# DoHoonKim8/stark-verifier

Hardware: AMD Instinct MI355X
Metric: recursive plonky2 proofs/sec (Semaphore d=20) (higher is better)
Workload: dtype u64 (Goldilocks field, integer); 1 GPU; recursive: per unit one Semaphore signal (group 2^20, n=2^13, blowup 8, 28 FRI queries, 16 PoW bits, zk) + the recursive proof verifying it (n=2^14, same FRI parameters); 128 units per GPU per step, 10 prover contexts per GPU; all_gather of (nullifier|topic) + Poseidon aggregation root per step; parallelism=independent proofs sharded over ranks, no data-path collective, exchange=none (one rank): gl355_aggregation_root over the local leaves, units_proven_in_process=1674

## Files before the change

stark-verifier_amd/csrc/gl355_internal.h:

```cpp
#pragma once
#include <hip/hip_runtime.h>
#include <stdint.h>
#include <string.h>

#include <algorithm>
#include <map>
#include <mutex>
#include <string>
#include <vector>

#include "../../include/gl355.h"
#include "gl_field.cuh"
#include "merkle_common.cuh"
#include "coset_interp.h"

namespace gl355 { struct Ctx; }

struct gl355_oracle {
    struct gl355::Ctx* ctx;
    uint32_t log_n, rate_bits, batch, leaf_len, cap_height;
    uint64_t* coeffs;
    uint64_t* lde;
    uint64_t* digests;
    uint64_t* cap;
    uint64_t n_digests;
    int32_t hasher;
};

namespace gl355 {

struct Ctx;

#define GL355_HIP(ctx, expr)                                                          \
    do {                                                                              \
        hipError_t _e = (expr);                                                       \
        if (_e != hipSuccess) return (ctx)->fail_hip(_e, #expr, __FILE__, __LINE__);  \
    } while (0)
#define GL355_TRY(expr)          \
    do {                         \
        int32_t _rc = (expr);    \
        if (_rc != GL355_OK) return _rc; \
    } while (0)
#define LAUNCH_CHECK(ctx) GL355_HIP(ctx, hipGetLastError())

struct Ctx {
    int device = 0;
    hipStream_t stream = nullptr;
    bool own_stream = false;
    bool external_stream = false;
    std::string err;
    uint64_t* tw_fwd = nullptr;
    uint64_t* tw_inv = nullptr;
    const uint64_t* twr(uint32_t rho, bool inv) const { return tw_fwd + 32768 + ((rho - 3) * 2 + (inv ? 1 : 0)) * 32768; }
    hipEvent_t ev0 = nullptr, ev1 = nullptr;

    struct PowTab { uint64_t* lo; uint64_t* hi; };
    std::map<std::vector<uint64_t>, PowTab> pow_cache;
    std::map<std::vector<uint64_t>, uint64_t*> full_cache;
    int32_t full_pow_table(const uint64_t* lo, const uint64_t* hi, uint32_t n_cosets, uint32_t log_n, const uint64_t** out);
    int32_t full_step_table(const uint64_t* lo, const uint64_t* hi, uint32_t l1, uint32_t l2, bool inv, const uint64_t** out);
    int32_t nat_step_table(const uint64_t* lo, const uint64_t* hi, uint32_t l1, uint32_t l2, const uint64_t** out);
    int32_t l24_mid_table(const uint64_t** out);

    struct Block { void* p; size_t size; bool used; uint64_t serial; };
    std::vector<Block> blocks;
    uint64_t block_serial = 0;

    struct ProfRec { const char* name; hipEvent_t e0, e1; uint64_t bytes; };
    uint32_t replay_threads = 1;
    uint32_t batch_units = 8;
    uint32_t ntt_single_pass_max_log = 12;
    int blocking_sync = 0;
    hipEvent_t sync_ev = nullptr;
    hipError_t wait();
    hipError_t wait_impl();
    hipError_t d2h(void* dst, const void* src, size_t bytes);
    uint64_t wait_ns = 0, wait_calls = 0;
    uint64_t wait_cpu_ns = 0, prove_cpu_ns = 0, prove_calls = 0;
    uint32_t merkle_lanes_log = 14;
    uint32_t leaf_lanes_log = 16;
    bool prof_on = false;
    std::vector<ProfRec> prof;
    std::vector<hipEvent_t> ev_pool;
    hipEvent_t prof_event();

    int32_t fail(int32_t code, const char* msg);
    int32_t fail_hip(hipError_t e, const char* expr, const char* file, int line);
    int32_t alloc(size_t bytes, void** out);
    void release(void* p);
    void* pinned_buf = nullptr;
    size_t pinned_size = 0;
    int32_t pinned(size_t bytes, void** out);
    void* rt_rows[2] = {nullptr, nullptr};
    void* rt_drows[2] = {nullptr, nullptr};
    void* rt_aux[2] = {nullptr, nullptr};
    size_t rt_bytes = 0, rt_aux_bytes = 0;
    bool device_replay = true;
    hipStream_t rt_copy_stream = nullptr;
    int32_t runtime_buffers(size_t bytes, size_t aux_bytes, uint64_t* rows[2], uint64_t* drows[2], void* aux[2], hipStream_t* copy_stream);
    void runtime_buffers_free();
    void release_all();
    void trim_since(uint64_t mark);
    int32_t pow_tables_multi(const std::vector<uint64_t>& bases, const uint64_t** lo, const uint64_t** hi);
    int32_t pow_tables(uint64_t base, const uint64_t** lo, const uint64_t** hi) {
        return pow_tables_multi(std::vector<uint64_t>{gl_canon(base)}, lo, hi);
    }
};

struct ProfScope {
    Ctx* ctx; int idx = -1;
    ProfScope(Ctx* c, const char* name, uint64_t alg_bytes = 0) : ctx(c) {
        if (!c->prof_on) return;
        Ctx::ProfRec r{name, c->prof_event(), c->prof_event(), alg_bytes};
        if (!r.e0 || !r.e1) return;
        (void)hipEventRecord(r.e0, c->stream);
// ... 264 lines not shown
```

stark-verifier_amd/csrc/merkle.hip:

```cpp
#include "gl355_internal.h"
#include "poseidon.cuh"
#include "merkle_common.cuh"

namespace gl355 {


struct PoseidonHasher {
    static constexpr bool wide_digests = true;
    static GL_DEV void permute(uint64_t (&s)[12]) { psd_permute(s); }
    static GL_DEV uint64_t out(uint64_t x) { return gl_canon(x); }
    static GL_DEV uint64_t in2(uint64_t x) { return x; }
};

__global__ void __launch_bounds__(256) poseidon_permute_kernel(uint64_t* states, uint64_t count) { permute_body<PoseidonHasher>(states, count); }

constexpr int psd_leaf_waves = 4;
__global__ void __launch_bounds__(256) __attribute__((amdgpu_waves_per_eu(psd_leaf_waves))) hash_leaves_kernel(LeafArgs a) { hash_leaves_body<PoseidonHasher>(a); }

__global__ void __launch_bounds__(256) merkle_level_kernel(uint64_t* digests, uint64_t* cap, uint32_t sub_bits,
                                                          uint32_t layer, uint64_t n_nodes ) {
    merkle_level_body<PoseidonHasher>(digests, cap, sub_bits, layer, n_nodes);
}

__device__ __constant__ const uint32_t PSD_CIRC_DEV[12] = {17, 15, 41, 16, 2, 28, 13, 13, 39, 18, 34, 20};
// ... 219 lines not shown
#undef GL355_WIDE_LEAVES
        GL355_HIP(ctx, hipGetLastError());
    }
    return merkle_build_above_leaves(ctx, n_groups, sub_bits, digests, cap);
}

int32_t merkle_build_above_leaves(Ctx* ctx, uint64_t n_leaves, uint32_t sub_bits, uint64_t* digests, uint64_t* cap) {
    const uint64_t lanes_max = 1ull << ctx->merkle_lanes_log;
    const uint32_t top_levels_max = (n_leaves >> sub_bits) < 64 ? 6 : MERKLE_TOP_LEVELS;
    const bool fast_lanes = (n_leaves >> sub_bits) < 64;
    uint32_t top_levels = std::min<uint32_t>(top_levels_max, sub_bits);
    while (top_levels > 1 && ((n_leaves >> (sub_bits - top_levels + 1)) > lanes_max)) top_levels--;
    uint32_t top_from = sub_bits + 1;
    if (top_levels >= 1 && ((n_leaves >> (sub_bits - top_levels + 1)) <= lanes_max)) top_from = sub_bits - top_levels + 1;
    for (uint32_t layer = 1; layer <= sub_bits; layer++) {
        const uint64_t n_nodes = n_leaves >> layer;
        if (layer == top_from) {
            ProfScope ps(ctx, "merkle_top_kernel", (2 * n_nodes - (n_leaves >> sub_bits)) * 96);
            if (fast_lanes) hipLaunchKernelGGL(merkle_top_kernel<3>, dim3((uint32_t)(n_leaves >> sub_bits)), dim3(1024), 0, ctx->stream, digests, cap, sub_bits, layer, top_levels);
            else hipLaunchKernelGGL(merkle_top_kernel<0>, dim3((uint32_t)(n_leaves >> sub_bits)), dim3(1024), 0, ctx->stream, digests, cap, sub_bits, layer, top_levels);
            GL355_HIP(ctx, hipGetLastError());
            break;
        }
        ProfScope ps(ctx, n_nodes <= lanes_max ? "merkle_level_lanes_kernel" : "merkle_level_kernel", n_nodes * 96);
        if (n_nodes <= lanes_max) {
            if (fast_lanes) hipLaunchKernelGGL(merkle_level_lanes_kernel<3>, dim3((uint32_t)((n_nodes + 3) / 4)), dim3(64), 0, ctx->stream,
                                               digests, cap, sub_bits, layer, n_nodes);
            else hipLaunchKernelGGL(merkle_level_lanes_kernel<0>, dim3((uint32_t)((n_nodes + 3) / 4)), dim3(64), 0, ctx->stream,
                                    digests, cap, sub_bits, layer, n_nodes);
        } else {
            hipLaunchKernelGGL(merkle_level_kernel, dim3((uint32_t)((n_nodes + 255) / 256)), dim3(256), 0, ctx->stream,
                               digests, cap, sub_bits, layer, n_nodes);
        }
        GL355_HIP(ctx, hipGetLastError());
    }
    return GL355_OK;
}

int32_t pow_grind_units_dev(Ctx* ctx, int32_t hasher, uint32_t B, const uint64_t* states, const uint32_t* pos, uint32_t bits, uint64_t start, uint64_t* landing,
                            uint64_t* const* witness_host) {
    if (bits > 40) return ctx->fail(GL355_E_UNSUPPORTED, "pow: more than 40 bits of grinding refused");
    const HasherLaunch& h = launch_of(hasher);
    PowArgs pa;
    memset(&pa, 0, sizeof pa);
    for (uint32_t u = 0; u < B; u++) {
        for (int k = 0; k < 12; k++) pa.state[u * 12 + k] = gl_canon(states[u * 12 + k]);
        pa.pos[u] = pos[u]; pa.todo[u] = 1;
    }
    Scratch pb(ctx);
    GL355_TRY(pb.get(GL355_MAX_UNITS * 8));
    pa.best = reinterpret_cast<unsigned long long*>(pb.p);
    pa.bits = bits;
    GL355_HIP(ctx, hipMemsetAsync(pb.p, 0xFF, GL355_MAX_UNITS * 8, ctx->stream));
    uint64_t per_launch = 1ull << std::min<uint32_t>(std::max<uint32_t>(bits + 1, 12), h.grind_window_log);
    uint64_t base = start;
    for (uint32_t left = B; left;) {
        ProfScope ps(ctx, h.grind_scope, 0);
        pa.start = base;
        hipLaunchKernelGGL(h.grind, dim3((uint32_t)(per_launch / 256), B), dim3(256), 0, ctx->stream, pa);
        GL355_HIP(ctx, hipGetLastError());
        GL355_HIP(ctx, ctx->d2h(landing, pb.p, (uint64_t)B * 8));
        GL355_HIP(ctx, ctx->wait());
        for (uint32_t u = 0; u < B; u++)
            if (pa.todo[u] && landing[u] != ~0ull) { *witness_host[u] = landing[u]; pa.todo[u] = 0; left--; }
        base += per_launch;
        if (per_launch < (1ull << h.grind_window_log)) per_launch <<= 1;
        if (base - start > (1ull << 44)) return ctx->fail(GL355_E_UNSUPPORTED, "pow: no witness found in 2^44 candidates");
    }
    return GL355_OK;
}

int32_t pow_grind_dev(Ctx* ctx, int32_t hasher, const uint64_t state[12], uint32_t pos, uint32_t bits, uint64_t start,
                      uint64_t* witness_host) {
    if (pos >= 8) return ctx->fail(GL355_E_INVALID_ARG, "pow: witness position must be in the rate part");
    uint64_t landing;
    return pow_grind_units_dev(ctx, hasher, 1, state, &pos, bits, start, &landing, &witness_host);
}

}
```

stark-verifier_amd/csrc/merkle_common.cuh:

```cuda
#pragma once
#include <stdint.h>
#include <hip/hip_runtime.h>

#include "../../include/gl355.h"
#include "gl_field.cuh"

namespace gl355 {

__host__ __device__ __forceinline__ uint64_t digest_slot(uint32_t layer, uint64_t k) {
    return 2 * (((k >> 1) << (layer + 1)) + (1ull << layer) - 1) + (k & 1);
}

__device__ __forceinline__ uint64_t* leaf_digest_dst(uint64_t* out, uint64_t* cap, uint32_t linear, uint32_t sub_bits, uint64_t i) {
    if (linear) return out + i * 4;
    if (sub_bits == 0) return cap + i * 4;
    const uint64_t sub_leaves = 1ull << sub_bits;
    const uint64_t t = i >> sub_bits, k = i & (sub_leaves - 1);
    return out + (t * 2 * (sub_leaves - 1) + digest_slot(0, k)) * 4;
}

struct MerkleNode {
    uint64_t* tree; uint64_t* cap; uint32_t sub_bits, layer; uint64_t t, k;
    __device__ __forceinline__ uint64_t child() const { return digest_slot(layer - 1, 2 * k); }
    __device__ __forceinline__ uint64_t* dst() const { return (layer == sub_bits) ? cap + t * 4 : tree + digest_slot(layer, k) * 4; }
};
__device__ __forceinline__ MerkleNode merkle_node(uint64_t* digests, uint64_t* cap, uint32_t sub_bits, uint32_t layer, uint64_t t, uint64_t k) {
    const uint64_t sub_leaves = 1ull << sub_bits;
    return {digests + t * 2 * (sub_leaves - 1) * 4, cap, sub_bits, layer, t, k};
}
__device__ __forceinline__ MerkleNode merkle_node(uint64_t* digests, uint64_t* cap, uint32_t sub_bits, uint32_t layer, uint64_t g) {
    const uint64_t per = (1ull << sub_bits) >> layer;
    return merkle_node(digests, cap, sub_bits, layer, g / per, g % per);
}

struct LeafArgs {
    const uint64_t* leaves;
    uint64_t n_leaves;
    uint32_t leaf_len;
    uint32_t col_major;
    uint64_t stride;
    uint64_t* out;
    uint32_t sub_bits;
    uint32_t linear;
    uint32_t always_hash;
    uint64_t* cap;
    uint32_t unit_log;
    uint32_t n_main;
    uint64_t unit_stride;
    const uint64_t* salt;
    uint64_t salt_unit_stride;
};

__device__ __forceinline__ uint64_t leaf_elem(const LeafArgs& a, uint64_t g, uint32_t k) {
    if (a.unit_log == 0) return a.col_major ? a.leaves[(uint64_t)k * a.stride + g] : a.leaves[g * a.stride + k];
    const uint64_t u = g >> a.unit_log, i = g & ((1ull << a.unit_log) - 1);
    if (k < a.n_main) {
        const uint64_t* base = a.leaves + u * a.unit_stride;
        return a.col_major ? base[(uint64_t)k * a.stride + i] : base[i * a.stride + k];
    }
    return a.salt[u * a.salt_unit_stride + (uint64_t)(k - a.n_main) * a.stride + i];
}

struct PowArgs { uint64_t state[GL355_MAX_UNITS * 12]; uint32_t pos[GL355_MAX_UNITS]; uint32_t todo[GL355_MAX_UNITS]; uint32_t bits; uint64_t start; unsigned long long* best; };

#if defined(__HIPCC__)
#define GL_WAVE_LDS_SYNC()                                      \
    do {                                                        \
        __builtin_amdgcn_fence(__ATOMIC_SEQ_CST, "wavefront");  \
        __builtin_amdgcn_wave_barrier();                        \
    } while (0)

template <class H> GL_DEV void store_digest(uint64_t* dst, const uint64_t (&d)[4]) {
    if constexpr (H::wide_digests) {
        *reinterpret_cast<ulonglong2*>(dst) = make_ulonglong2(d[0], d[1]);
        *reinterpret_cast<ulonglong2*>(dst + 2) = make_ulonglong2(d[2], d[3]);
    } else {
#pragma unroll
        for (int k = 0; k < 4; k++) dst[k] = d[k];
    }
}

template <class H> GL_DEV void permute_body(uint64_t* states, uint64_t count) {
    const uint64_t i = blockIdx.x * (uint64_t)blockDim.x + threadIdx.x;
    if (i >= count) return;
    uint64_t s[12];
#pragma unroll
    for (int k = 0; k < 12; k++) s[k] = states[i * 12 + k];
    H::permute(s);
#pragma unroll
    for (int k = 0; k < 12; k++) states[i * 12 + k] = H::out(s[k]);
}

template <class H> GL_DEV void hash_leaves_body(const LeafArgs& a) {
    const uint64_t i = blockIdx.x * (uint64_t)blockDim.x + threadIdx.x;
    if (i >= a.n_leaves) return;
    uint64_t s[12];
#pragma unroll
    for (int k = 0; k < 12; k++) s[k] = 0;
    const uint32_t len = a.leaf_len;
    uint64_t d[4];
    if (len <= 4 && !a.always_hash) {
        for (uint32_t k = 0; k < 4; k++) {
            uint64_t v = 0;
            if (k < len) v = leaf_elem(a, i, k);
            d[k] = gl_canon(v);
        }
    } else {
#pragma unroll 1
        for (uint32_t off = 0; off < len; off += 8) {
            const uint32_t m = min(8u, len - off);
#pragma unroll
            for (uint32_t k = 0; k < 8; k++) {
                if (k < m) s[k] = leaf_elem(a, i, off + k);
            }
            H::permute(s);
        }
#pragma unroll
        for (int k = 0; k < 4; k++) d[k] = H::out(s[k]);
    }
    store_digest<H>(leaf_digest_dst(a.out, a.cap, a.linear, a.sub_bits, i), d);
}

template <class H> GL_DEV void merkle_level_body(uint64_t* digests, uint64_t* cap, uint32_t sub_bits, uint32_t layer, uint64_t n_nodes ) {
    const uint64_t g = blockIdx.x * (uint64_t)blockDim.x + threadIdx.x;
    if (g >= n_nodes) return;
    const MerkleNode nd = merkle_node(digests, cap, sub_bits, layer, g);
    const uint64_t* in = nd.tree + nd.child() * 4;
    uint64_t s[12];
    if constexpr (H::wide_digests) {
        const ulonglong2 l0 = *reinterpret_cast<const ulonglong2*>(in);
        const ulonglong2 l1 = *reinterpret_cast<const ulonglong2*>(in + 2);
        const ulonglong2 r0 = *reinterpret_cast<const ulonglong2*>(in + 4);
        const ulonglong2 r1 = *reinterpret_cast<const ulonglong2*>(in + 6);
        s[0] = l0.x; s[1] = l0.y; s[2] = l1.x; s[3] = l1.y; s[4] = r0.x; s[5] = r0.y; s[6] = r1.x; s[7] = r1.y;
    } else {
#pragma unroll
        for (int e = 0; e < 8; e++) s[e] = in[e];
    }
#pragma unroll
    for (int e = 8; e < 12; e++) s[e] = 0;
    H::permute(s);
    const uint64_t d[4] = {H::out(s[0]), H::out(s[1]), H::out(s[2]), H::out(s[3])};
    store_digest<H>(nd.dst(), d);
}

template <class H> GL_DEV void two_to_one_body(const uint64_t* l, const uint64_t* r, uint64_t n, uint64_t* out) {
    const uint64_t i = blockIdx.x * (uint64_t)blockDim.x + threadIdx.x;
    if (i >= n) return;
    uint64_t s[12] = {H::in2(l[4 * i]), H::in2(l[4 * i + 1]), H::in2(l[4 * i + 2]), H::in2(l[4 * i + 3]),
                      H::in2(r[4 * i]), H::in2(r[4 * i + 1]), H::in2(r[4 * i + 2]), H::in2(r[4 * i + 3]), 0, 0, 0, 0};
    H::permute(s);
#pragma unroll
    for (int k = 0; k < 4; k++) out[4 * i + k] = H::out(s[k]);
}

template <class H> GL_DEV void pow_grind_units_body(const PowArgs& a) {
    const uint32_t u = blockIdx.y;
    if (!a.todo[u]) return;
    const uint64_t w = a.start + blockIdx.x * (uint64_t)blockDim.x + threadIdx.x;
    if (w > __hip_atomic_load(a.best + u, __ATOMIC_RELAXED, __HIP_MEMORY_SCOPE_AGENT)) return;
    uint64_t s[12];
#pragma unroll
    for (int k = 0; k < 12; k++) s[k] = a.state[u * 12 + k];
#pragma unroll
    for (int k = 0; k < 12; k++) if ((uint32_t)k == a.pos[u]) s[k] = w;
    H::permute(s);
    const uint64_t resp = H::out(s[7]);
    if (a.bits == 0 || (resp >> (64 - a.bits)) == 0) atomicMin(a.best + u, (unsigned long long)w);
}
#endif

}
```

stark-verifier_amd/csrc/prover_batch.hip:

```cpp
#include "gl355_internal.h"
#include "blinding.cuh"
#include "poseidon.cuh"

using namespace gl355;

namespace gl355 {

struct BOracle {
    Ctx* ctx = nullptr;
    uint32_t B = 0, log_n = 0, rate_bits = 0, batch = 0, leaf_len = 0, cap_height = 0;
    uint64_t* base = nullptr;
    uint64_t *coeffs = nullptr, *lde = nullptr, *salt = nullptr, *digests = nullptr, *cap = nullptr;
    uint64_t n_dig = 0;
    ~BOracle() { if (base && ctx) ctx->release(base); }
    int32_t alloc(Ctx* c, uint32_t b, uint32_t lg, uint32_t rb, uint32_t bat, bool salted, uint32_t cap_h) {
        ctx = c; B = b; log_n = lg; rate_bits = rb; batch = bat; leaf_len = bat + (salted ? GL355_SALT_SIZE : 0); cap_height = cap_h;
        const uint64_t n = 1ull << lg, N = n << rb, n_cap = 1ull << cap_h;
        n_dig = 2 * (N - n_cap);
        const uint64_t total = (uint64_t)B * ((uint64_t)bat * n + (uint64_t)leaf_len * N + n_dig * 4 + n_cap * 4);
        void* p = nullptr;
        GL355_TRY(c->alloc(total * 8, &p));
        base = reinterpret_cast<uint64_t*>(p);
        coeffs = base;
        lde = coeffs + (uint64_t)B * bat * n;
// ... 14 lines not shown

struct UnitKeys { BlindKey k[MAXB]; };

__global__ void witness_rows_units_kernel(uint64_t* wires, uint64_t n, uint32_t num_wires, const uint32_t* row_idx, const uint64_t* row_vals,
                                          uint32_t n_rows) {
    const uint64_t g = blockIdx.x * (uint64_t)blockDim.x + threadIdx.x;
    const uint64_t per = (uint64_t)n_rows * num_wires;
    if (g >= per) return;
    const uint32_t u = blockIdx.y, r = g / num_wires, c = g % num_wires;
    wires[((uint64_t)u * num_wires + c) * n + row_idx[r]] = gl_canon(row_vals[(uint64_t)u * per + g]);
}
__global__ void witness_blind_units_kernel(uint64_t* wires, uint64_t n, uint32_t num_wires, uint32_t num_routed, uint32_t blind_start, uint32_t n_blind,
                                           uint32_t z_start, uint32_t n_z_pairs, UnitKeys keys) {
    const uint64_t b = blockIdx.x * (uint64_t)blockDim.x + threadIdx.x;
    const uint64_t n_a = (uint64_t)n_blind * num_wires, n_z = (uint64_t)n_z_pairs * num_routed;
    if (4 * b >= n_a + n_z) return;
    const uint32_t u = blockIdx.y;
    uint64_t* w = wires + (uint64_t)u * num_wires * n;
    uint64_t e[4];
    blind_block_elements(keys.k[u], GL355_BLIND_STREAM_WITNESS, (uint32_t)b, e);
#pragma unroll
    for (int j = 0; j < 4; j++) {
        const uint64_t g = 4 * b + j;
        if (g < n_a) {
            const uint32_t c = g / n_blind, r = g % n_blind;
            w[(uint64_t)c * n + blind_start + r] = e[j];
        } else if (g < n_a + n_z) {
            const uint64_t h = g - n_a, c = h / n_z_pairs, k = h % n_z_pairs;
            w[c * n + z_start + 2 * k] = e[j];
            w[c * n + z_start + 2 * k + 1] = e[j];
        }
    }
}
__global__ void salt_units_kernel(uint64_t* salt, uint32_t lde_bits, UnitKeys keys, uint32_t stream) {
    const uint64_t b = blockIdx.x * (uint64_t)blockDim.x + threadIdx.x;
    const uint64_t N = 1ull << lde_bits, cnt = (uint64_t)GL355_SALT_SIZE * N;
    if (4 * b >= cnt) return;
    const uint32_t u = blockIdx.y;
    uint64_t e[4];
    blind_block_elements(keys.k[u], stream, (uint32_t)b, e);
#pragma unroll
    for (int j = 0; j < 4; j++) {
        const uint64_t g = 4 * b + j;
        const uint64_t c = g >> lde_bits, i = g & (N - 1);
        const uint64_t r = __brevll(i) >> (64 - lde_bits);
        salt[((uint64_t)u * GL355_SALT_SIZE + c) * N + r] = e[j];
    }
}

struct ZsArgs {
    const uint64_t* wires; uint64_t wires_us;
    const uint64_t* sigmas; const uint64_t* k_is;
    uint32_t log_n, n_routed, max_degree, nch, n_chunks, npp;
    uint64_t g;
    uint64_t* chunk_q;
    uint64_t* row_prod;
    uint64_t* zbuf; uint64_t z_us;
    UnitVals betas, gammas;
};
constexpr int ZS_MAX_CHUNKS = 16;
__global__ void __launch_bounds__(256) zs_rows_units_kernel(ZsArgs a) {
    const uint64_t n = 1ull << a.log_n;
    const uint64_t i = blockIdx.x * (uint64_t)blockDim.x + threadIdx.x;
    if (i >= n) return;
    const uint32_t inst = blockIdx.y, u = inst / a.nch, k = inst % a.nch;
    const uint64_t beta = a.betas.v[u * 4 + k], gamma = a.gammas.v[u * 4 + k];
    const uint64_t* wires = a.wires + (uint64_t)u * a.wires_us;
    const uint64_t x = gl_pow(a.g, i);
    const uint64_t bx = gl_mul(beta, x);
    uint64_t num[ZS_MAX_CHUNKS], pre[ZS_MAX_CHUNKS], den[ZS_MAX_CHUNKS];
    uint64_t run = 1;
#pragma unroll
    for (int ch = 0; ch < ZS_MAX_CHUNKS; ch++) {
        num[ch] = 1; den[ch] = 1; pre[ch] = run;
        if ((uint32_t)ch < a.n_chunks) {
            uint64_t nm = 1, dn = 1;
            for (uint32_t j = ch * a.max_degree; j < (ch + 1) * a.max_degree && j < a.n_routed; j++) {
                const uint64_t w = wires[(uint64_t)j * n + i];
                nm = gl_mul(nm, gl_add(gl_add(w, gl_mul(bx, a.k_is[j])), gamma));
                dn = gl_mul(dn, gl_add(gl_add(w, gl_mul(beta, a.sigmas[(uint64_t)j * n + i])), gamma));
            }
            num[ch] = nm; den[ch] = dn;
            run = gl_mul(run, dn);
        }
    }
    uint64_t inv = gl_inv(run);
    uint64_t rp = 1;
    uint64_t* cq = a.chunk_q + (uint64_t)inst * a.n_chunks * n;
#pragma unroll
    for (int ch = ZS_MAX_CHUNKS - 1; ch >= 0; ch--) {
        if ((uint32_t)ch < a.n_chunks) {
            const uint64_t dinv = gl_mul(inv, pre[ch]);
            inv = gl_mul(inv, den[ch]);
            const uint64_t q = gl_mul(num[ch], dinv);
            cq[(uint64_t)ch * n + i] = q;
            rp = gl_mul(rp, q);
        }
    }
    a.row_prod[(uint64_t)inst * n + i] = rp;
}
__global__ void __launch_bounds__(1024) zs_scan_units_kernel(ZsArgs a) {
    __shared__ uint64_t sh[1024];
    const int tid = threadIdx.x;
    const uint32_t inst = blockIdx.x, u = inst / a.nch, k = inst % a.nch;
    const uint64_t n = 1ull << a.log_n;
    const uint64_t* row_prod = a.row_prod + (uint64_t)inst * n;
    uint64_t* z = a.zbuf + (uint64_t)u * a.z_us + (uint64_t)k * n;
    uint64_t running = 1;
    for (uint64_t base = 0; base < n; base += 1024) {
        const uint64_t i = base + tid;
        uint64_t v = i < n ? row_prod[i] : 1;
        sh[tid] = v;
        __syncthreads();
        for (int s = 1; s < 1024; s <<= 1) {
            uint64_t o = tid >= s ? sh[tid - s] : 1;
            __syncthreads();
            v = gl_mul(v, o);
            sh[tid] = v;
            __syncthreads();
        }
        const uint64_t excl = tid ? sh[tid - 1] : 1;
// ... 7 lines not shown
    const uint64_t n = 1ull << a.log_n;
    const uint64_t i = blockIdx.x * (uint64_t)blockDim.x + threadIdx.x;
    if (i >= n) return;
    const uint32_t inst = blockIdx.y, u = inst / a.nch, k = inst % a.nch;
    uint64_t* zu = a.zbuf + (uint64_t)u * a.z_us;
    const uint64_t* cq = a.chunk_q + (uint64_t)inst * a.n_chunks * n;
    uint64_t* pp = zu + ((uint64_t)a.nch + (uint64_t)k * a.npp) * n;
    uint64_t acc = zu[(uint64_t)k * n + i];
    for (uint32_t ch = 0; ch + 1 < a.n_chunks; ch++) {
        acc = gl_mul(acc, cq[(uint64_t)ch * n + i]);
        pp[(uint64_t)ch * n + i] = gl_canon(acc);
    }
}

static int32_t commit_units(Ctx* ctx, int32_t hasher, BOracle& o, bool is_coeffs, bool canonical, const UnitKeys* keys, uint32_t stream_id) {
    const uint64_t n = 1ull << o.log_n, N = n << o.rate_bits;
    const uint32_t cols = o.B * o.batch, lde_bits = o.log_n + o.rate_bits;
    if (!is_coeffs) GL355_TRY(ntt_dev(ctx, o.coeffs, o.log_n, cols, n, true, 0));
    else if (!canonical) GL355_TRY(canon_dev(ctx, o.coeffs, (uint64_t)cols * n));
    GL355_TRY(lde_dev(ctx, o.coeffs, n, o.log_n, o.rate_bits, GL355_COSET_SHIFT, cols, o.lde, N, true));
    if (o.salt) {
        const uint64_t cnt = (uint64_t)GL355_SALT_SIZE * N;
        ProfScope ps(ctx, "salt", cnt * 8 * o.B);
        hipLaunchKernelGGL(salt_units_kernel, dim3((uint32_t)((cnt / 4 + 255) / 256), o.B), dim3(256), 0, ctx->stream, o.salt, lde_bits, *keys, stream_id);
        LAUNCH_CHECK(ctx);
    }
    LeafArgs a;
    memset(&a, 0, sizeof a);
    a.leaves = o.lde; a.n_leaves = (uint64_t)o.B * N; a.leaf_len = o.leaf_len; a.col_major = 1; a.stride = N;
    a.unit_log = lde_bits; a.n_main = o.batch; a.unit_stride = (uint64_t)o.batch * N; a.salt = o.salt; a.salt_unit_stride = (uint64_t)GL355_SALT_SIZE * N;
    return merkle_build_args(ctx, hasher, a, lde_bits - o.cap_height, o.digests, o.cap);
}

int32_t observe_caps_units(Ctx* ctx, uint32_t B, uint64_t n_cap, const uint64_t* d_caps, uint64_t* stage, gl355_challenger* ch, uint64_t* const* dst) {
    GL355_HIP(ctx, ctx->d2h(stage, d_caps, (uint64_t)B * n_cap * 32));
    GL355_HIP(ctx, ctx->wait());
    for (uint32_t u = 0; u < B; u++) {
        memcpy(dst[u], stage + (uint64_t)u * n_cap * 4, n_cap * 32);
        gl355_challenger_observe(&ch[u], dst[u], n_cap * 4);
    }
    return GL355_OK;
}

static int32_t zs_units_dev(Ctx* ctx, uint32_t B, uint32_t nch, const uint64_t* wires, uint64_t wires_us, const uint64_t* sigmas, const uint64_t* k_is,
                            uint32_t log_n, uint32_t routed, uint32_t max_degree, const UnitVals& betas, const UnitVals& gammas, uint64_t* zbuf, uint64_t z_us) {
    const uint64_t n = 1ull << log_n;
    const uint32_t n_inst = B * nch, n_chunks = (routed + max_degree - 1) / max_degree;
    Scratch zs_tmp(ctx);
    GL355_TRY(zs_tmp.get((uint64_t)n_inst * (n_chunks + 1) * n * 8));
    ZsArgs za;
    memset(&za, 0, sizeof za);
    za.wires = wires; za.wires_us = wires_us; za.sigmas = sigmas; za.k_is = k_is;
    za.log_n = log_n; za.n_routed = routed; za.max_degree = max_degree; za.nch = nch; za.n_chunks = n_chunks; za.npp = n_chunks - 1;
    za.g = gl_root_of_unity(log_n);
    za.chunk_q = zs_tmp.as<uint64_t>(); za.row_prod = za.chunk_q + (uint64_t)n_inst * n_chunks * n;
    za.zbuf = zbuf; za.z_us = z_us;
    for (uint32_t i = 0; i < MAXB * 4; i++) { za.betas.v[i] = gl_canon(betas.v[i]); za.gammas.v[i] = gl_canon(gammas.v[i]); }
    ProfScope ps(ctx, "zs_partial_products", (uint64_t)n_inst * ((uint64_t)routed * n * 16 + (uint64_t)n_chunks * n * 8));
    const uint32_t blocks = (uint32_t)((n + 255) / 256);
    hipLaunchKernelGGL(zs_rows_units_kernel, dim3(blocks, n_inst), dim3(256), 0, ctx->stream, za);
    LAUNCH_CHECK(ctx);
    hipLaunchKernelGGL(zs_scan_units_kernel, dim3(n_inst), dim3(1024), 0, ctx->stream, za);
    LAUNCH_CHECK(ctx);
    hipLaunchKernelGGL(zs_partials_units_kernel, dim3(blocks, n_inst), dim3(256), 0, ctx->stream, za);
    LAUNCH_CHECK(ctx);
    return GL355_OK;
}
int32_t zs_partial_products_dev(Ctx* ctx, const uint64_t* wires, const uint64_t* sigmas, const uint64_t* k_is, uint32_t log_n, uint32_t n_routed,
                                uint32_t max_degree, uint64_t beta, uint64_t gamma, uint64_t* z_out, uint64_t* pp_out) {
    const uint64_t n = 1ull << log_n;
    const uint32_t n_chunks = (n_routed + max_degree - 1) / max_degree;
    if (n_chunks > ZS_MAX_CHUNKS) return ctx->fail(GL355_E_UNSUPPORTED, "zs_partial_products: at most 16 partial-product chunks");
    Scratch zb(ctx);
    GL355_TRY(zb.get((uint64_t)n_chunks * n * 8));
    UnitVals betas, gammas;
    memset(&betas, 0, sizeof betas); memset(&gammas, 0, sizeof gammas);
    betas.v[0] = beta; gammas.v[0] = gamma;
    GL355_TRY(zs_units_dev(ctx, 1, 1, wires, 0, sigmas, k_is, log_n, n_routed, max_degree, betas, gammas, zb.as<uint64_t>(), (uint64_t)n_chunks * n));
    GL355_HIP(ctx, hipMemcpyAsync(z_out, zb.p, n * 8, hipMemcpyDeviceToDevice, ctx->stream));
    if (n_chunks > 1) GL355_HIP(ctx, hipMemcpyAsync(pp_out, zb.as<uint64_t>() + n, (uint64_t)(n_chunks - 1) * n * 8, hipMemcpyDeviceToDevice, ctx->stream));
    return GL355_OK;
}

struct ProveRun {
    Ctx* ctx; const gl355_prover_data* pd; const gl355_circuit& c; const gl355_oracle* cs; const ProveUnit* io;
    const uint32_t B, nch, qdf, npp, routed, nw, z_width, lde_bits, cap_h, L, nq_idx;
    const uint64_t n, N, n_cap;
    const int32_t hasher; const bool zk;
    const ProofLayout lay;
    std::vector<gl355_challenger> ch;
    std::vector<uint64_t*> out;
    std::vector<uint64_t> q_idx;
    UnitKeys keys;
    UnitVals pi_hashes;
    uint64_t* stage = nullptr;
    BOracle o_w, o_z, o_q;
    OView views[4];
    PolySet all, zsset;
    UnitVals betas, gammas, alphas, zetas, fri_alpha;
    Scratch wires_keep;
    Staged s_sig, s_k;
    Scratch evb, colsA, colsB, fri_vals, ob;
    uint64_t *d_idx = nullptr, *d_open = nullptr;
    uint64_t off_leaf[4], off_sib[4], off_ev = 0, off_fsib = 0, open_words = 0;

    ProveRun(Ctx* cx, const gl355_prover_data* p, uint32_t b, const ProveUnit* units)
        : ctx(cx), pd(p), c(*p->circuit), cs(p->constants_sigmas), io(units), B(b), nch(c.num_challenges), qdf(c.max_degree), npp(c.num_partial_products),
// ... 274 lines not shown
```

stark-verifier_amd/csrc/quotient.hip:

```cpp
#include "gl355_internal.h"
#include "poseidon.cuh"

namespace gl355 {

struct QuotArgs {
    gl355_circuit c;
    const uint64_t* cs;
    const uint64_t* wires;
    const uint64_t* zs;
    uint64_t lde_stride;
    uint32_t qbits;
    const uint64_t* k_is;
    const uint64_t* xw_lo;
    const uint64_t* xw_hi;
    uint64_t zh_inv[16];
    uint64_t zh[16];
    uint64_t n_inv;
    uint64_t* out;
    const uint64_t* alpha_pw;
    uint32_t pw_stride;
    uint64_t wires_us, zs_us;
    uint64_t betas[GL355_MAX_UNITS * 4], gammas[GL355_MAX_UNITS * 4], pi_hash[GL355_MAX_UNITS * 4];
};

typedef const __attribute__((address_space(4))) uint64_t* PwTable;
template <int NCH>
struct AlphaAcc {
    uint64_t acc[NCH];
    PwTable tab;
    uint32_t stride, idx;
    GL_DEV void init(const QuotArgs& a, uint32_t unit, uint32_t first = 0) {
#pragma unroll
        for (int c = 0; c < NCH; c++) acc[c] = 0;
        tab = (PwTable)(a.alpha_pw + (uint64_t)unit * NCH * a.pw_stride); stride = a.pw_stride; idx = first;
    }
    GL_DEV void push(uint64_t term) {
#pragma unroll
        for (int c = 0; c < NCH; c++) acc[c] = gl_add(acc[c], gl_mul(term, tab[c * stride + idx]));
        idx++;
    }
    GL_DEV void push_at(uint64_t term, uint32_t k) {
#pragma unroll
        for (int c = 0; c < NCH; c++) acc[c] = gl_add(acc[c], gl_mul(term, tab[c * stride + k]));
    }
};
template <int NCH>
struct LazyAcc : AlphaAcc<NCH> {
    GL_DEV uint64_t value(int c) const { return this->acc[c]; }
};
template <>
struct LazyAcc<2> {
    uint64_t A0[2], A1[2], A2[2];
    uint32_t k0[2], k1[2], k2[2];
    PwTable tab;
    uint32_t stride, idx;
    GL_DEV void init(const QuotArgs& a, uint32_t unit, uint32_t first = 0) {
#pragma unroll
        for (int c = 0; c < 2; c++) { A0[c] = A1[c] = A2[c] = 0; k0[c] = k1[c] = k2[c] = 0; }
        tab = (PwTable)(a.alpha_pw + (uint64_t)unit * 2 * a.pw_stride); stride = a.pw_stride; idx = first;
    }
    GL_DEV void push(uint64_t term) {
        const uint64_t ax = tab[idx], ay = tab[stride + idx];
        const uint32_t t0 = (uint32_t)term, t1 = (uint32_t)(term >> 32);
        uint64_t c0, c1, c2, c3;
        asm("v_mad_u64_u32 %0, %12, %16, %18, %0\n\t"
            "v_mad_u64_u32 %1, %13, %16, %20, %1\n\t"
            "v_mad_u64_u32 %2, %14, %16, %19, %2\n\t"
            "v_mad_u64_u32 %3, %15, %16, %21, %3\n\t"
            "v_addc_co_u32_e64 %6, vcc, 0, %6, %12\n\t"
            "v_addc_co_u32_e64 %7, vcc, 0, %7, %13\n\t"
// ... 339 lines not shown
    uint32_t brk = s.degree, ni = 0;
    for (uint32_t i0 = 0; i0 < s.n; i0 += 4) {
        uint64_t v[8];
#pragma unroll
        for (int k = 0; k < 8; k++) v[k] = nx[k];
        wire_group<8>(w, 1 + 2 * (i0 + 4), last, nx);
#pragma unroll
        for (int k = 0; k < 4; k++) {
            const uint32_t i = i0 + k;
            if (i == brk) {
                uint64_t ie[2], ip[2];
                wire_group<2>(w, s.start_int + 2 * ni, s.start_int + 2 * ni + 1, ie);
                wire_group<2>(w, s.start_int + 2 * (s.n_int + ni), s.start_int + 2 * (s.n_int + ni) + 1, ip);
                push2(g, gl2_sub(gl2_make(ie[0], ie[1]), eval));
                push2(g, gl2_sub(gl2_make(ip[0], ip[1]), prod));
                eval = gl2_make(ie[0], ie[1]); prod = gl2_make(ip[0], ip[1]);
                ni++; brk += s.degree - 1;
            }
            const gl2 xm = gl2_make(gl_sub(x.c0, xs[i * stride]), x.c1);
            const gl2 vw = gl2_mul_base(gl2_make(v[2 * k], v[2 * k + 1]), ws[i]);
            eval = gl2_add(gl2_mul(eval, xm), gl2_mul(vw, prod));
            prod = gl2_mul(prod, xm);
        }
    }
    push2(g, gl2_sub(gl2_make(pv[2], pv[3]), eval));
}

template <int NCH, bool STAGE = false, bool INTERP = false>
__global__ void __launch_bounds__(STAGE ? 64 : 128) __attribute__((amdgpu_waves_per_eu(STAGE ? 1 : 3, 3))) quotient_kernel(QuotArgs a) {
    extern __shared__ __attribute__((aligned(16))) uint64_t wire_lds[];
    const uint64_t nq = 1ull << a.qbits;
    const uint64_t t = blockIdx.x * (uint64_t)blockDim.x + threadIdx.x;
    if (t >= nq) return;
    const uint32_t unit = blockIdx.y;
    const uint64_t* __restrict__ wglob = a.wires + (uint64_t)unit * a.wires_us;
    WireSrc w{wglob, a.lde_stride, t, a.lde_stride};
    if constexpr (STAGE) {
        for (uint32_t j = 0; j < a.c.num_wires; j++) wire_lds[j * 64 + threadIdx.x] = wglob[(uint64_t)j * a.lde_stride + t];
        w = WireSrc{wire_lds, 64, threadIdx.x, a.lde_stride};
    }
    const uint64_t* __restrict__ zs = a.zs + (uint64_t)unit * a.zs_us;
    const uint32_t qdb = a.qbits - a.c.degree_bits;
    const uint64_t iq = __brevll(t) >> (64 - a.qbits);
    const uint64_t x = gl_mul_small(gl_mul(a.xw_lo[iq & 4095], a.xw_hi[iq >> 12]), 7);
    const uint64_t iq_next = (iq + (1ull << qdb)) & (nq - 1);
    const uint64_t t_next = __brevll(iq_next) >> (64 - a.qbits);
    constexpr uint32_t nch = NCH;
    const uint32_t npp = a.c.num_partial_products;
    const uint32_t routed = a.c.num_routed_wires, chunk = a.c.max_degree;
    const uint32_t n_sel = a.c.num_selectors, n_cst = a.c.num_constants;

    AlphaAcc<NCH> total;
    total.init(a, unit);
    const uint64_t zh = a.zh[iq & ((1u << qdb) - 1)];
    const uint64_t l0 = gl_mul(gl_mul(zh, a.n_inv), gl_inv(gl_sub(x, 1)));
    for (uint32_t c = 0; c < nch; c++) {
        const uint64_t z = zs[(uint64_t)c * a.lde_stride + t];
        total.push(gl_sub(gl_mul(l0, z), l0));
    }
    {
        const uint32_t n_chunks = (routed + chunk - 1) / chunk;
        uint64_t prev[NCH], bx[NCH];
#pragma unroll
        for (int c = 0; c < NCH; c++) {
            prev[c] = zs[(uint64_t)c * a.lde_stride + t];
            bx[c] = gl_mul(a.betas[unit * 4 + c], x);
        }
        const uint32_t first = total.idx;
        const uint32_t sig0 = n_sel + n_cst;
        uint64_t wn = WIRE(0), sn = CONST(sig0), kn = a.k_is[0];
        for (uint32_t ch = 0; ch < n_chunks; ch++) {
            uint64_t num[NCH], den[NCH];
#pragma unroll
            for (int c = 0; c < NCH; c++) { num[c] = 1; den[c] = 1; }
            for (uint32_t j = ch * chunk; j < (ch + 1) * chunk && j < routed; j++) {
                const uint64_t wj = wn, sj = sn, kj = kn;
                const uint32_t jn = j + 1 < routed ? j + 1 : routed - 1;
                wn = WIRE(jn); sn = CONST(sig0 + jn); kn = a.k_is[jn];
                if constexpr (NCH == 2) {
                    const uint64_t a1[4] = {bx[0], bx[1], a.betas[unit * 4], a.betas[unit * 4 + 1]}, b1[4] = {kj, kj, sj, sj};
                    uint64_t p1[4], p2[4];
                    gl_mul_multi<4>(a1, b1, p1);
                    const uint64_t wg0 = gl_add(wj, a.gammas[unit * 4]), wg1 = gl_add(wj, a.gammas[unit * 4 + 1]);
                    const uint64_t a2[4] = {num[0], num[1], den[0], den[1]};
                    const uint64_t b2[4] = {gl_add(wg0, p1[0]), gl_add(wg1, p1[1]), gl_add(wg0, p1[2]), gl_add(wg1, p1[3])};
                    gl_mul_multi<4>(a2, b2, p2);
                    num[0] = p2[0]; num[1] = p2[1]; den[0] = p2[2]; den[1] = p2[3];
                } else {
#pragma unroll
                    for (int c = 0; c < NCH; c++) {
                        const uint64_t wg = gl_add(wj, a.gammas[unit * 4 + c]);
                        num[c] = gl_mul(num[c], gl_add(wg, gl_mul(bx[c], kj)));
                        den[c] = gl_mul(den[c], gl_add(wg, gl_mul(a.betas[unit * 4 + c], sj)));
                    }
                }
            }
#pragma unroll
            for (int c = 0; c < NCH; c++) {
                const uint64_t next = (ch + 1 < n_chunks) ? zs[(uint64_t)(nch + c * npp + ch) * a.lde_stride + t]
                                                          : zs[(uint64_t)c * a.lde_stride + t_next];
                total.push_at(gl_sub(gl_mul(prev[c], num[c]), gl_mul(next, den[c])), first + c * n_chunks + ch);
                prev[c] = next;
            }
        }
        total.idx = first + nch * n_chunks;
    }
    uint64_t gate_sum[NCH];
#pragma unroll
    for (int c = 0; c < NCH; c++) gate_sum[c] = 0;
    for (uint32_t gi = 0; gi < a.c.num_gates; gi++) {
        const gl355_gate gt = a.c.gates[gi];
        if (gt.type == GL355_GATE_NOOP) continue;
        GateAccT<NCH> g;
        WireSrc wg = w;
        uint64_t tg = t;
        asm volatile("" : "+s"(wg.stride), "+s"(wg.cs_stride), "+v"(tg));
        wg.idx = STAGE ? w.idx : tg;
        g.init(a, unit, total.idx);
        bool interp = false;
        if constexpr (INTERP) {
            if (gt.type == GL355_GATE_COSET_INTERPOLATION) { gate_coset_interpolation(a, wg, tg, g, gt.param); interp = true; }
        }
        if (!interp) switch (gt.type) {
            case GL355_GATE_POSEIDON: gate_poseidon(a, wg, tg, g); break;
            case GL355_GATE_BASE_SUM: gate_base_sum(a, wg, tg, g, gt.param); break;
            case GL355_GATE_CONSTANT: gate_constant(a, wg, tg, g, gt.param); break;
            case GL355_GATE_PUBLIC_INPUT: gate_public_input(a, wg, tg, g, unit); break;
            case GL355_GATE_ARITHMETIC: gate_arithmetic(a, wg, tg, g, gt.param); break;
            case GL355_GATE_ARITHMETIC_EXT: gate_arithmetic_ext(a, wg, tg, g, gt.param); break;
            case GL355_GATE_MUL_EXT: gate_mul_ext(a, wg, tg, g, gt.param); break;
            case GL355_GATE_POSEIDON_MDS: gate_poseidon_mds(a, wg, tg, g); break;
            case GL355_GATE_RANDOM_ACCESS: gate_random_access(a, wg, tg, g, gt.param); break;
            case GL355_GATE_REDUCING: gate_reducing<false>(a, wg, tg, g, gt.param); break;
            case GL355_GATE_REDUCING_EXT: gate_reducing<true>(a, wg, tg, g, gt.param); break;
            default: break;
        }
        const uint64_t sel = CONST(gt.selector_index);
        uint64_t filter = 1;
        for (uint32_t k = gt.group_start; k < gt.group_end; k++)
            if (k != gi) filter = gl_mul(filter, gl_sub(k, sel));
        if (n_sel > 1) filter = gl_mul(filter, gl_sub(0xFFFFFFFFull, sel));
#pragma unroll
        for (uint32_t c = 0; c < nch; c++) gate_sum[c] = gl_add(gate_sum[c], gl_mul(filter, g.value(c)));
    }
    const uint64_t zh_inv = a.zh_inv[iq & ((1u << qdb) - 1)];
    for (uint32_t c = 0; c < nch; c++) {
        const uint64_t v = gl_mul(gl_add(total.acc[c], gate_sum[c]), zh_inv);
        a.out[((uint64_t)unit * nch + c) * nq + t] = gl_canon(v);
    }
}

int32_t quotient_dev(Ctx* ctx, const gl355_circuit* c, const uint64_t* cs_lde, const uint64_t* wires_lde,
                     const uint64_t* zs_lde, uint64_t lde_stride, const uint64_t* k_is_dev, const uint64_t* betas,
                     const uint64_t* gammas, const uint64_t* alphas, const uint64_t pi_hash[4], uint64_t* out_values) {
    uint64_t b[4] = {0, 0, 0, 0}, g[4] = {0, 0, 0, 0}, al[4] = {0, 0, 0, 0};
    for (uint32_t i = 0; i < c->num_challenges && i < 4; i++) { b[i] = betas[i]; g[i] = gammas[i]; al[i] = alphas[i]; }
    return quotient_units_dev(ctx, c, 1, cs_lde, wires_lde, 0, zs_lde, 0, lde_stride, k_is_dev, b, g, al, pi_hash, out_values);
}

int32_t quotient_units_dev(Ctx* ctx, const gl355_circuit* c, uint32_t B, const uint64_t* cs_lde, const uint64_t* wires_lde, uint64_t wires_us,
                           const uint64_t* zs_lde, uint64_t zs_us, uint64_t lde_stride, const uint64_t* k_is_dev, const uint64_t* betas,
                           const uint64_t* gammas, const uint64_t* alphas, const uint64_t* pi_hashes, uint64_t* out_values) {
    uint32_t qdb = 0;
    while ((1u << qdb) < c->max_degree) qdb++;
    if ((1u << qdb) != c->max_degree || qdb > c->rate_bits || qdb > 4) return ctx->fail(GL355_E_UNSUPPORTED, "quotient: degree factor must be a power of two <= 2^rate_bits");
    if (c->num_challenges == 0 || c->num_challenges > 4) return ctx->fail(GL355_E_UNSUPPORTED, "quotient: 1..4 challenges");
    if (c->num_gates > GL355_MAX_GATES) return ctx->fail(GL355_E_INVALID_ARG, "quotient: too many gates");
    if (B == 0 || B > GL355_MAX_UNITS) return ctx->fail(GL355_E_INVALID_ARG, "quotient: 1..GL355_MAX_UNITS units");
    QuotArgs a;
    memset(&a, 0, sizeof a);
    a.c = *c;
    a.cs = cs_lde; a.wires = wires_lde; a.zs = zs_lde; a.lde_stride = lde_stride; a.wires_us = wires_us; a.zs_us = zs_us;
    a.qbits = c->degree_bits + qdb;
    a.k_is = k_is_dev;
    GL355_TRY(ctx->pow_tables(gl_root_of_unity(a.qbits), &a.xw_lo, &a.xw_hi));
    const uint64_t sn = gl_pow(7, 1ull << c->degree_bits);
    const uint64_t wq = gl_root_of_unity(qdb);
    uint64_t w = 1;
    for (uint32_t k = 0; k < (1u << qdb); k++) {
        a.zh[k] = gl_canon(gl_sub(gl_mul(sn, w), 1));
        a.zh_inv[k] = gl_canon(gl_inv(a.zh[k]));
        w = gl_mul(w, wq);
    }
    AlphaTabArgs ta;
    memset(&ta, 0, sizeof ta);
    for (uint32_t u = 0; u < B; u++) {
        for (uint32_t i = 0; i < c->num_challenges; i++) {
            a.betas[u * 4 + i] = gl_canon(betas[u * 4 + i]); a.gammas[u * 4 + i] = gl_canon(gammas[u * 4 + i]);
            ta.alphas[u * 4 + i] = gl_canon(alphas[u * 4 + i]);
        }
        for (int i = 0; i < 4; i++) a.pi_hash[u * 4 + i] = gl_canon(pi_hashes[u * 4 + i]);
    }
    a.n_inv = gl_canon(gl_inv((1ull << c->degree_bits) % GL_P));
    a.out = out_values;
    uint32_t longest = 0;
    bool has_interp = false;
    for (uint32_t g = 0; g < c->num_gates; g++) {
        const uint32_t p = c->gates[g].param;
        if (c->gates[g].type == GL355_GATE_RANDOM_ACCESS && ((p & 0xFF) < 1 || (p & 0xFF) > 4))
            return ctx->fail(GL355_E_UNSUPPORTED, "quotient: RandomAccessGate with 1..4 bits");
        uint32_t k = 0;
        if (c->gates[g].type == GL355_GATE_COSET_INTERPOLATION) {
            CosetInterpShape s;
            if ((p & 0xFF) < 2 || (p & 0xFF) > 4) return ctx->fail(GL355_E_UNSUPPORTED, "quotient: CosetInterpolationGate with 2..4 subgroup bits");
            if (!coset_interp_shape(p, s)) return ctx->fail(GL355_E_INVALID_ARG, "quotient: CosetInterpolationGate degree outside 2..2^subgroup_bits");
            if (s.num_wires > c->num_wires || s.start_int > c->num_routed_wires)
                return ctx->fail(GL355_E_INVALID_ARG, "quotient: CosetInterpolationGate does not fit the wires / routed wires");
            k = s.num_constraints;
            has_interp = true;
        }
        switch (c->gates[g].type) {
            case GL355_GATE_CONSTANT: k = p; break;
            case GL355_GATE_PUBLIC_INPUT: k = 4; break;
            case GL355_GATE_BASE_SUM: k = 1 + p; break;
            case GL355_GATE_POSEIDON: k = 123; break;
            case GL355_GATE_ARITHMETIC: k = p; break;
            case GL355_GATE_ARITHMETIC_EXT: case GL355_GATE_MUL_EXT: case GL355_GATE_REDUCING: case GL355_GATE_REDUCING_EXT: k = 2 * p; break;
            case GL355_GATE_POSEIDON_MDS: k = 24; break;
            case GL355_GATE_RANDOM_ACCESS: k = ((p >> 8) & 0xFF) * ((p & 0xFF) + 2) + ((p >> 16) & 0xFF); break;
            default: break;
        }
        longest = k > longest ? k : longest;
    }
    const uint32_t n_chunks = (c->num_routed_wires + c->max_degree - 1) / c->max_degree;
    a.pw_stride = ((c->num_challenges * (1 + n_chunks) + longest + 1) + 63) & ~63u;
    Scratch pw(ctx);
    GL355_TRY(pw.get((size_t)B * c->num_challenges * a.pw_stride * 8));
    a.alpha_pw = pw.as<uint64_t>();
    ta.nch = c->num_challenges; ta.stride = a.pw_stride; ta.out = pw.as<uint64_t>();
    hipLaunchKernelGGL(alpha_table_kernel, dim3((a.pw_stride + 255) / 256, B), dim3(256), 0, ctx->stream, ta);
    GL355_HIP(ctx, hipGetLastError());
    const uint64_t nq = 1ull << a.qbits;
    ProfScope ps(ctx, "quotient_kernel", (uint64_t)B * nq * 8 * ((uint64_t)c->num_selectors + c->num_constants + c->num_routed_wires + c->num_wires +
                                                   (uint64_t)c->num_challenges * (2 + c->num_partial_products)));
    const dim3 grid((uint32_t)((nq + 127) / 128), B);
    if (has_interp) {
        switch (c->num_challenges) {
            case 1: hipLaunchKernelGGL((quotient_kernel<1, false, true>), grid, dim3(128), 0, ctx->stream, a); break;
            case 2: hipLaunchKernelGGL((quotient_kernel<2, false, true>), grid, dim3(128), 0, ctx->stream, a); break;
            case 3: hipLaunchKernelGGL((quotient_kernel<3, false, true>), grid, dim3(128), 0, ctx->stream, a); break;
            default: hipLaunchKernelGGL((quotient_kernel<4, false, true>), grid, dim3(128), 0, ctx->stream, a); break;
        }
    } else switch (c->num_challenges) {
        case 1: hipLaunchKernelGGL(quotient_kernel<1>, grid, dim3(128), 0, ctx->stream, a); break;
        case 2: hipLaunchKernelGGL(quotient_kernel<2>, grid, dim3(128), 0, ctx->stream, a); break;
        case 3: hipLaunchKernelGGL(quotient_kernel<3>, grid, dim3(128), 0, ctx->stream, a); break;
// ... 8 lines not shown
```

Baseline: 328.2 recursive proofs/s.

## Cache L0 and root powers in tables, and grid-stride the PoW grind kernel

The quotient kernel now reads a cached per-coset-point L0 table instead of computing a field inverse per point. The Z/partial-product kernel uses two-level power tables instead of gl_pow per row. The PoW grind kernel becomes grid-stride with a capped grid and larger windows, which cuts per-launch overhead and host round trips. These are three unrelated ideas. They cost extra table memory and cache lookups, and the larger grind windows may do wasted work after a witness is found.

```diff
diff --git a/stark-verifier_amd/csrc/gl355_internal.h b/stark-verifier_amd/csrc/gl355_internal.h
--- a/stark-verifier_amd/csrc/gl355_internal.h
+++ b/stark-verifier_amd/csrc/gl355_internal.h
@@ -61,6 +61,7 @@
     int32_t full_step_table(const uint64_t* lo, const uint64_t* hi, uint32_t l1, uint32_t l2, bool inv, const uint64_t** out);
     int32_t nat_step_table(const uint64_t* lo, const uint64_t* hi, uint32_t l1, uint32_t l2, const uint64_t** out);
     int32_t l24_mid_table(const uint64_t** out);
+    int32_t l0_table(uint32_t degree_bits, uint32_t qbits, const uint64_t* xw_lo, const uint64_t* xw_hi, const uint64_t zh[16], const uint64_t** out);
 
     struct Block { void* p; size_t size; bool used; uint64_t serial; };
     std::vector<Block> blocks;
diff --git a/stark-verifier_amd/csrc/merkle.hip b/stark-verifier_amd/csrc/merkle.hip
--- a/stark-verifier_amd/csrc/merkle.hip
+++ b/stark-verifier_amd/csrc/merkle.hip
@@ -295,12 +295,14 @@
     pa.best = reinterpret_cast<unsigned long long*>(pb.p);
     pa.bits = bits;
     GL355_HIP(ctx, hipMemsetAsync(pb.p, 0xFF, GL355_MAX_UNITS * 8, ctx->stream));
-    uint64_t per_launch = 1ull << std::min<uint32_t>(std::max<uint32_t>(bits + 1, 12), h.grind_window_log);
+    uint64_t per_launch = 1ull << std::min<uint32_t>(std::max<uint32_t>(bits + 3, 12), h.grind_window_log);
+    constexpr uint32_t GRIND_WGS = 256;
+    const uint32_t G = B == 1 ? 512 : 1u << (log2_u64(std::max<uint32_t>(GRIND_WGS / B, 16) + 1) - 1);
     uint64_t base = start;
     for (uint32_t left = B; left;) {
         ProfScope ps(ctx, h.grind_scope, 0);
-        pa.start = base;
-        hipLaunchKernelGGL(h.grind, dim3((uint32_t)(per_launch / 256), B), dim3(256), 0, ctx->stream, pa);
+        pa.start = base; pa.window = (uint32_t)per_launch;
+        hipLaunchKernelGGL(h.grind, dim3((uint32_t)std::min<uint64_t>(per_launch / 256, G), B), dim3(256), 0, ctx->stream, pa);
         GL355_HIP(ctx, hipGetLastError());
         GL355_HIP(ctx, ctx->d2h(landing, pb.p, (uint64_t)B * 8));
         GL355_HIP(ctx, ctx->wait());
diff --git a/stark-verifier_amd/csrc/merkle_common.cuh b/stark-verifier_amd/csrc/merkle_common.cuh
--- a/stark-verifier_amd/csrc/merkle_common.cuh
+++ b/stark-verifier_amd/csrc/merkle_common.cuh
@@ -61,7 +61,7 @@
     return a.salt[u * a.salt_unit_stride + (uint64_t)(k - a.n_main) * a.stride + i];
 }
 
-struct PowArgs { uint64_t state[GL355_MAX_UNITS * 12]; uint32_t pos[GL355_MAX_UNITS]; uint32_t todo[GL355_MAX_UNITS]; uint32_t bits; uint64_t start; unsigned long long* best; };
+struct PowArgs { uint64_t state[GL355_MAX_UNITS * 12]; uint32_t pos[GL355_MAX_UNITS]; uint32_t todo[GL355_MAX_UNITS]; uint32_t bits, window; uint64_t start; unsigned long long* best; };
 
 #if defined(__HIPCC__)
 #define GL_WAVE_LDS_SYNC()                                      \
@@ -157,16 +157,21 @@
 template <class H> GL_DEV void pow_grind_units_body(const PowArgs& a) {
     const uint32_t u = blockIdx.y;
     if (!a.todo[u]) return;
-    const uint64_t w = a.start + blockIdx.x * (uint64_t)blockDim.x + threadIdx.x;
-    if (w > __hip_atomic_load(a.best + u, __ATOMIC_RELAXED, __HIP_MEMORY_SCOPE_AGENT)) return;
-    uint64_t s[12];
+    const uint32_t step = gridDim.x * blockDim.x;
+    for (uint32_t off = blockIdx.x * blockDim.x + threadIdx.x; off < a.window; off += step) {
+        const uint64_t w = a.start + off;
+        if (w > __hip_atomic_load(a.best + u, __ATOMIC_RELAXED, __HIP_MEMORY_SCOPE_AGENT)) return;
+        uint32_t us = u;
+        asm volatile("" : "+s"(us));
+        uint64_t s[12];
 #pragma unroll
-    for (int k = 0; k < 12; k++) s[k] = a.state[u * 12 + k];
+        for (int k = 0; k < 12; k++) s[k] = a.state[us * 12 + k];
 #pragma unroll
-    for (int k = 0; k < 12; k++) if ((uint32_t)k == a.pos[u]) s[k] = w;
-    H::permute(s);
-    const uint64_t resp = H::out(s[7]);
-    if (a.bits == 0 || (resp >> (64 - a.bits)) == 0) atomicMin(a.best + u, (unsigned long long)w);
+        for (int k = 0; k < 12; k++) if ((uint32_t)k == a.pos[us]) s[k] = w;
+        H::permute(s);
+        const uint64_t resp = H::out(s[7]);
+        if (a.bits == 0 || (resp >> (64 - a.bits)) == 0) atomicMin(a.best + u, (unsigned long long)w);
+    }
 }
 #endif
 
diff --git a/stark-verifier_amd/csrc/prover_batch.hip b/stark-verifier_amd/csrc/prover_batch.hip
--- a/stark-verifier_amd/csrc/prover_batch.hip
+++ b/stark-verifier_amd/csrc/prover_batch.hip
@@ -90,7 +90,7 @@
     const uint64_t* wires; uint64_t wires_us;
     const uint64_t* sigmas; const uint64_t* k_is;
     uint32_t log_n, n_routed, max_degree, nch, n_chunks, npp;
-    uint64_t g;
+    const uint64_t* g_lo; const uint64_t* g_hi;
     uint64_t* chunk_q;
     uint64_t* row_prod;
     uint64_t* zbuf; uint64_t z_us;
@@ -104,7 +104,7 @@
     const uint32_t inst = blockIdx.y, u = inst / a.nch, k = inst % a.nch;
     const uint64_t beta = a.betas.v[u * 4 + k], gamma = a.gammas.v[u * 4 + k];
     const uint64_t* wires = a.wires + (uint64_t)u * a.wires_us;
-    const uint64_t x = gl_pow(a.g, i);
+    const uint64_t x = gl_mul(a.g_lo[i & 4095], a.g_hi[i >> 12]);
     const uint64_t bx = gl_mul(beta, x);
     uint64_t num[ZS_MAX_CHUNKS], pre[ZS_MAX_CHUNKS], den[ZS_MAX_CHUNKS];
     uint64_t run = 1;
@@ -218,7 +218,8 @@
     memset(&za, 0, sizeof za);
     za.wires = wires; za.wires_us = wires_us; za.sigmas = sigmas; za.k_is = k_is;
     za.log_n = log_n; za.n_routed = routed; za.max_degree = max_degree; za.nch = nch; za.n_chunks = n_chunks; za.npp = n_chunks - 1;
-    za.g = gl_root_of_unity(log_n);
+    if (log_n > 24) return ctx->fail(GL355_E_UNSUPPORTED, "zs_partial_products: at most 2^24 rows (the two-level power table)");
+    GL355_TRY(ctx->pow_tables(gl_root_of_unity(log_n), &za.g_lo, &za.g_hi));
     za.chunk_q = zs_tmp.as<uint64_t>(); za.row_prod = za.chunk_q + (uint64_t)n_inst * n_chunks * n;
     za.zbuf = zbuf; za.z_us = z_us;
     for (uint32_t i = 0; i < MAXB * 4; i++) { za.betas.v[i] = gl_canon(betas.v[i]); za.gammas.v[i] = gl_canon(gammas.v[i]); }
diff --git a/stark-verifier_amd/csrc/quotient.hip b/stark-verifier_amd/csrc/quotient.hip
--- a/stark-verifier_amd/csrc/quotient.hip
+++ b/stark-verifier_amd/csrc/quotient.hip
@@ -15,7 +15,7 @@
     const uint64_t* xw_hi;
     uint64_t zh_inv[16];
     uint64_t zh[16];
-    uint64_t n_inv;
+    const uint64_t* l0;
     uint64_t* out;
     const uint64_t* alpha_pw;
     uint32_t pw_stride;
@@ -461,8 +461,7 @@
 
     AlphaAcc<NCH> total;
     total.init(a, unit);
-    const uint64_t zh = a.zh[iq & ((1u << qdb) - 1)];
-    const uint64_t l0 = gl_mul(gl_mul(zh, a.n_inv), gl_inv(gl_sub(x, 1)));
+    const uint64_t l0 = a.l0[t];
     for (uint32_t c = 0; c < nch; c++) {
         const uint64_t z = zs[(uint64_t)c * a.lde_stride + t];
         total.push(gl_sub(gl_mul(l0, z), l0));
@@ -557,6 +556,37 @@
         const uint64_t v = gl_mul(gl_add(total.acc[c], gate_sum[c]), zh_inv);
         a.out[((uint64_t)unit * nch + c) * nq + t] = gl_canon(v);
     }
+}
+
+struct L0TabArgs { const uint64_t* xw_lo; const uint64_t* xw_hi; uint32_t qbits, qdb; uint64_t zh[16]; uint64_t n_inv; uint64_t* out; };
+__global__ void __launch_bounds__(256) l0_table_kernel(L0TabArgs a) {
+    const uint64_t t = blockIdx.x * (uint64_t)blockDim.x + threadIdx.x;
+    if (t >= (1ull << a.qbits)) return;
+    const uint64_t iq = __brevll(t) >> (64 - a.qbits);
+    const uint64_t x = gl_mul_small(gl_mul(a.xw_lo[iq & 4095], a.xw_hi[iq >> 12]), 7);
+    const uint64_t zh = a.zh[iq & ((1u << a.qdb) - 1)];
+    a.out[t] = gl_canon(gl_mul(gl_mul(zh, a.n_inv), gl_inv(gl_sub(x, 1))));
+}
+int32_t Ctx::l0_table(uint32_t degree_bits, uint32_t qbits, const uint64_t* xw_lo, const uint64_t* xw_hi, const uint64_t zh[16], const uint64_t** out) {
+    const std::vector<uint64_t> key{6, degree_bits, qbits};
+    auto it = full_cache.find(key);
+    if (it != full_cache.end()) { *out = it->second; return GL355_OK; }
+    const uint64_t nq = 1ull << qbits;
+    L0TabArgs ta;
+    memset(&ta, 0, sizeof ta);
+    ta.xw_lo = xw_lo; ta.xw_hi = xw_hi; ta.qbits = qbits; ta.qdb = qbits - degree_bits;
+    for (uint32_t k = 0; k < (1u << ta.qdb); k++) ta.zh[k] = zh[k];
+    ta.n_inv = gl_canon(gl_inv((1ull << degree_bits) % GL_P));
+    uint64_t* d = nullptr;
+    GL355_HIP(this, hipMalloc((void**)&d, nq * 8));
+    ta.out = d;
+    hipLaunchKernelGGL(l0_table_kernel, dim3((uint32_t)((nq + 255) / 256)), dim3(256), 0, stream, ta);
+    const hipError_t launched = hipGetLastError();
+    if (launched != hipSuccess) (void)hipFree(d);
+    GL355_HIP(this, launched);
+    full_cache[key] = d;
+    *out = d;
+    return GL355_OK;
 }
 
 int32_t quotient_dev(Ctx* ctx, const gl355_circuit* c, const uint64_t* cs_lde, const uint64_t* wires_lde,
@@ -600,7 +630,7 @@
         }
         for (int i = 0; i < 4; i++) a.pi_hash[u * 4 + i] = gl_canon(pi_hashes[u * 4 + i]);
     }
-    a.n_inv = gl_canon(gl_inv((1ull << c->degree_bits) % GL_P));
+    GL355_TRY(ctx->l0_table(c->degree_bits, a.qbits, a.xw_lo, a.xw_hi, a.zh, &a.l0));
     a.out = out_values;
     uint32_t longest = 0;
     bool has_interp = false;
```

Measured after the change: 331.3 recursive proofs/s (median of 6 runs). No clear change (+0.9%).
